# pearl-robot-lab/2HandedAfforder

Hardware: AMD Instinct MI355X
Metric: affordance frames/sec/GPU @1024^2, 32-tok prompt; mask IoU vs ref (higher is better)
Workload: dtype bf16; 1 GPU; BASELINE.json configs[2]: 2HandedAfforder-7B, 64 x 1024x1024 uint8 NHWC frames/step/GPU, 32-token prompt (T=291), 8 forced answer tokens with [SEG], KV-cached greedy decode, random-init weights; CLIP + SAM preprocessing of the uint8 frames on the device inside the step; parallelism=frame-sharded replicas x1 (no collective), hip_streams=2, fp32_decoder_tail=True, fp32_residual_stream=off, neck_f32=False, sam_chunk=16, sam_waits_for_prefill=False, decode_chain=False

## Files before the change

### 2handedafforder_amd/csrc/attention.hip

```cpp
#include "haff_common.h"

#include <type_traits>

namespace {

struct AttnArgs {
  const bf16_t *q = nullptr, *k = nullptr, *v = nullptr;
  bf16_t* o = nullptr;
  long q_sb = 0, q_sh = 0, q_st = 0;
  long k_sb = 0, k_sh = 0, k_st = 0;
  long v_sb = 0, v_sh = 0, v_st = 0;
  long o_sb = 0, o_sh = 0, o_st = 0;
  int B = 0, H = 0, Nq = 0, Nk = 0, d = 0;
  float scale = 0.f;
  int q_pos0 = 0;
  const float *relh = nullptr, *relw = nullptr;
  int S = 0;
  const int* nk_rows = nullptr;
  const bf16_t *knew = nullptr, *vnew = nullptr;
  const float* cos_sin = nullptr;
  const bf16_t *tab_h = nullptr, *tab_w = nullptr;
  float* lse = nullptr;
};
static_assert(std::is_trivially_copyable<AttnArgs>::value && sizeof(AttnArgs) == 240, "AttnArgs is passed to the kernels by value");

constexpr int QB = 128;
constexpr int KT = 64;
constexpr float LOG2E = 1.4426950408889634f;

typedef __attribute__((address_space(3))) bf16x4* lds_v4_ptr;


template <int DP, int BIAS, bool CAUSAL, int NDT = DP / 16, bool LSUM = false, bool FULL = false, bool F16 = false>
__global__ __launch_bounds__(256, 2) void attn_fwd_kernel(AttnArgs p) {
  using E = h16<F16>;
  static_assert(!FULL || (!CAUSAL && BIAS != 3), "FULL tiles only");
  constexpr int KSTRIDE = (DP * 2) % 64 == 32 ? DP * 2 : DP * 2 + 32;
  constexpr int VSTRIDE = DP * 2 + 32;
  constexpr int NCH = DP / 32;
  constexpr int CPR = DP / 8;
  constexpr int ND = NDT;
  constexpr int NKD = DP / 32;
  constexpr int SMAX = 32;
  constexpr int RSTRIDE = 2 * SMAX + 1;

  extern __shared__ __attribute__((aligned(16))) unsigned char smem_raw[];
  constexpr int STAGE_BYTES = KT * KSTRIDE + KT * VSTRIDE;
  unsigned char* sKV = smem_raw;
  float* sRel = reinterpret_cast<float*>(smem_raw + 2 * STAGE_BYTES);

  const int tid = threadIdx.x;
  const int lane = tid & 63;
  const int wave = tid >> 6;
  const int fr = lane & 15, fh = lane >> 4;
  const int nqb = (p.Nq + QB - 1) / QB;
  const int nbh = p.B * p.H;
  int bh_id, qblk;
  {
    const int id = blockIdx.x;
    if ((nbh & 7) == 0) {
      bh_id = (id & 7) + 8 * (id / (8 * nqb));
      qblk = (id >> 3) % nqb;
    } else {
      bh_id = id / nqb;
      qblk = id - bh_id * nqb;
    }
  }
  const int b = bh_id / p.H, h = bh_id - b * p.H;
  const int q0 = qblk * QB;
  const int Nk = p.nk_rows ? min(p.nk_rows[b], p.Nk) : p.Nk;

  const bf16_t* qb = p.q + (long)b * p.q_sb + (long)h * p.q_sh;
  const bf16_t* kb = p.k + (long)b * p.k_sb + (long)h * p.k_sh;
  const bf16_t* vb = p.v + (long)b * p.v_sb + (long)h * p.v_sh;

  const float sl2 = p.scale * LOG2E;
  bf16x8 qf[2][NKD];
  int qrow[2];
#pragma unroll
  for (int qt = 0; qt < 2; ++qt) {
    const int qi = q0 + wave * 32 + qt * 16 + fr;
    qrow[qt] = qi;
    const int qc = min(qi, p.Nq - 1);
#pragma unroll
    for (int kd = 0; kd < NKD; ++kd) {
      const int col = kd * 32 + fh * 8;
      uint4 r = make_uint4(0, 0, 0, 0);
      if (col < p.d) {
        float qv[8];
        load8h<F16>(qb + (long)qc * p.q_st + col, qv);
#pragma unroll
        for (int j = 0; j < 8; ++j) qv[j] *= sl2;
        r.x = E::pack2(qv[0], qv[1]); r.y = E::pack2(qv[2], qv[3]);
        r.z = E::pack2(qv[4], qv[5]); r.w = E::pack2(qv[6], qv[7]);
      }
      qf[qt][kd] = __builtin_bit_cast(bf16x8, r);
    }
  }

  const float inv_S = p.S > 0 ? 1.0f / (float)p.S : 0.f;
  float relw_r[2][4][4];
  const float* relh_row[2];
  if (BIAS == 2) {
    const long bh = (long)b * p.H + h;
#pragma unroll
    for (int qt = 0; qt < 2; ++qt) {
      const int qc = min(qrow[qt], p.Nq - 1);
      const float* rw = p.relw + (bh * p.Nq + qc) * p.S;
      relh_row[qt] = p.relh + (bh * p.Nq + qc) * p.S;
#pragma unroll
      for (int t = 0; t < 4; ++t) {
        float4 f = *reinterpret_cast<const float4*>(rw + 16 * t + 4 * fh);
        relw_r[qt][t][0] = f.x * LOG2E; relw_r[qt][t][1] = f.y * LOG2E;
        relw_r[qt][t][2] = f.z * LOG2E; relw_r[qt][t][3] = f.w * LOG2E;
      }
    }
  }
  float relh3[2][16], relw3[2][4];
  bool kw_ok[4];
  if (BIAS == 3) {
    const long bh = (long)b * p.H + h;
#pragma unroll
    for (int r = 0; r < 4; ++r) kw_ok[r] = (4 * fh + r) < p.S;
#pragma unroll
    for (int qt = 0; qt < 2; ++qt) {
      const int qc = min(qrow[qt], p.Nq - 1);
      const float* rh = p.relh + (bh * p.Nq + qc) * p.S;
      const float* rw = p.relw + (bh * p.Nq + qc) * p.S;
#pragma unroll
      for (int j = 0; j < 16; ++j) relh3[qt][j] = rh[min(j, p.S - 1)] * LOG2E;
#pragma unroll
      for (int r = 0; r < 4; ++r) relw3[qt][r] = rw[min(4 * fh + r, p.S - 1)] * LOG2E;
    }
  }
  if (BIAS == 1) {
    const long bh = (long)b * p.H + h;
    for (int i = tid; i < QB * 2 * p.S; i += 256) {
      const int ql = i / (2 * p.S);
      const int j = i - ql * 2 * p.S;
      const int qc = min(q0 + ql, p.Nq - 1);
      const float val = (j < p.S) ? p.relh[(bh * p.Nq + qc) * p.S + j] : p.relw[(bh * p.Nq + qc) * p.S + (j - p.S)];
      sRel[ql * RSTRIDE + j] = val * LOG2E;
    }
  }

  float relh_next[2] = {0.f, 0.f};
  if (BIAS == 2) {
    relh_next[0] = relh_row[0][0];
    relh_next[1] = relh_row[1][0];
  }

  int st_row[NCH], st_c[NCH];
#pragma unroll
  for (int i = 0; i < NCH; ++i) {
    const int id = tid + i * 256;
    st_row[i] = id / CPR;
    st_c[i] = id - st_row[i] * CPR;
  }
  uint4 kreg[NCH], vreg[NCH];
#pragma unroll
  for (int i = 0; i < NCH; ++i) kreg[i] = vreg[i] = make_uint4(0, 0, 0, 0);
  const bf16_t* kptr[NCH];
  const bf16_t* vptr[NCH];
  bool col_ok[NCH];
#pragma unroll
  for (int i = 0; i < NCH; ++i) {
    col_ok[i] = st_c[i] * 8 < p.d;
    kptr[i] = kb + (long)st_row[i] * p.k_st + st_c[i] * 8;
    vptr[i] = vb + (long)st_row[i] * p.v_st + st_c[i] * 8;
  }
  const long k_step = (long)KT * p.k_st, v_step = (long)KT * p.v_st;
  auto load_tile = [&](int kt) {
    const bool plain = FULL || ((BIAS != 3) && (kt * KT + KT <= Nk));
#pragma unroll
    for (int i = 0; i < NCH; ++i) {
      if (col_ok[i]) {
        if (plain) {
          kreg[i] = *reinterpret_cast<const uint4*>(kptr[i] + kt * k_step);
          vreg[i] = *reinterpret_cast<const uint4*>(vptr[i] + kt * v_step);
        } else {
          int key = kt * KT + st_row[i];
          if (BIAS == 3) key = min(key >> 4, p.S - 1) * p.S + min(key & 15, p.S - 1);
          key = min(key, Nk - 1);
          kreg[i] = *reinterpret_cast<const uint4*>(kb + (long)key * p.k_st + st_c[i] * 8);
          vreg[i] = *reinterpret_cast<const uint4*>(vb + (long)key * p.v_st + st_c[i] * 8);
        }
      }
    }
  };
  auto write_tile = [&](int buf) {
    unsigned char* wK = sKV + buf * STAGE_BYTES;
    unsigned char* wV = wK + KT * KSTRIDE;
#pragma unroll
    for (int i = 0; i < NCH; ++i) {
      if (col_ok[i]) {
        *reinterpret_cast<uint4*>(wK + st_row[i] * KSTRIDE + st_c[i] * 16) = kreg[i];
        *reinterpret_cast<uint4*>(wV + st_row[i] * VSTRIDE + st_c[i] * 16) = vreg[i];
      }
    }
  };
#pragma unroll
  for (int i = 0; i < NCH; ++i) {
    if (!col_ok[i]) {
      uint4 vpad = make_uint4(0, 0, 0, 0);
      if (LSUM && st_c[i] * 8 == p.d) vpad.x = F16 ? 0x3c00u : 0x3f80u;
#pragma unroll
      for (int b2 = 0; b2 < 2; ++b2) {
        unsigned char* wK = sKV + b2 * STAGE_BYTES;
        unsigned char* wV = wK + KT * KSTRIDE;
        *reinterpret_cast<uint4*>(wK + st_row[i] * KSTRIDE + st_c[i] * 16) = make_uint4(0, 0, 0, 0);
        *reinterpret_cast<uint4*>(wV + st_row[i] * VSTRIDE + st_c[i] * 16) = vpad;
      }
    }
  }

  f32x4 oacc[ND][2];
#pragma unroll
  for (int dt = 0; dt < ND; ++dt) {
    oacc[dt][0] = f32x4{0.f, 0.f, 0.f, 0.f};
    oacc[dt][1] = f32x4{0.f, 0.f, 0.f, 0.f};
  }
  float m_run[2] = {0.f, 0.f};
  float l_run[2] = {0.f, 0.f};

  int nkt = (Nk + KT - 1) / KT;
  if (BIAS == 3) nkt = (16 * p.S + KT - 1) / KT;
  if (CAUSAL) {
    const int last_q = min(q0 + QB - 1, p.Nq - 1);
    const int last_key = min(last_q + p.q_pos0, Nk - 1);
    nkt = min(nkt, last_key / KT + 1);
  }

  load_tile(0);
  write_tile(0);
  __syncthreads();
  for (int kt = 0; kt < nkt; ++kt) {
    const unsigned char* sK = sKV + (kt & 1) * STAGE_BYTES;
    const unsigned char* sV = sK + KT * KSTRIDE;
    float rh_cur[2] = {relh_next[0], relh_next[1]};
    if (BIAS == 2) asm volatile("" : "+v"(rh_cur[0]), "+v"(rh_cur[1]));
    if (kt + 1 < nkt) load_tile(kt + 1);

    f32x4 sacc[4][2];
#pragma unroll
    for (int qt = 0; qt < 2; ++qt) {
      float rh3[4] = {0.f, 0.f, 0.f, 0.f};
      if (BIAS == 3) {
#pragma unroll
        for (int j = 0; j < 4; ++j)
          rh3[j] = kt == 0 ? relh3[qt][j] : (kt == 1 ? relh3[qt][4 + j] : (kt == 2 ? relh3[qt][8 + j] : relh3[qt][12 + j]));
      }
      const float msub = m_run[qt];
      const float rhv = rh_cur[qt] * LOG2E - msub;
#pragma unroll
      for (int t = 0; t < 4; ++t) {
        if (BIAS == 2) sacc[t][qt] = f32x4{relw_r[qt][t][0] + rhv, relw_r[qt][t][1] + rhv, relw_r[qt][t][2] + rhv, relw_r[qt][t][3] + rhv};
        else if (BIAS == 3) {
          const float rb = rh3[t] - msub;
          sacc[t][qt] = f32x4{relw3[qt][0] + rb, relw3[qt][1] + rb, relw3[qt][2] + rb, relw3[qt][3] + rb};
        }
        else sacc[t][qt] = f32x4{-msub, -msub, -msub, -msub};
      }
      if (BIAS == 2 && kt + 1 < nkt) relh_next[qt] = relh_row[qt][kt + 1];
    }
#pragma unroll
    for (int kd = 0; kd < NKD; ++kd) {
#pragma unroll
      for (int t = 0; t < 4; ++t) {
        const bf16x8 kf = *reinterpret_cast<const bf16x8*>(sK + (16 * t + fr) * KSTRIDE + (kd * 4 + fh) * 16);
        sacc[t][0] = E::mfma16(kf, qf[0][kd], sacc[t][0]);
        sacc[t][1] = E::mfma16(kf, qf[1][kd], sacc[t][1]);
      }
    }

    bool need_mask = !FULL && (kt * KT + KT > Nk);
    if (CAUSAL) need_mask = need_mask || (kt * KT + KT - 1 > q0 + wave * 32 + p.q_pos0);
    int off_h[4][4], off_w[4][4];
    if (BIAS == 1) {
#pragma unroll
      for (int t = 0; t < 4; ++t)
#pragma unroll
        for (int r = 0; r < 4; ++r) {
          const int kc = min(kt * KT + 16 * t + 4 * fh + r, Nk - 1);
          const int kh = (int)(((float)kc + 0.5f) * inv_S);
          off_h[t][r] = kh;
          off_w[t][r] = p.S + kc - kh * p.S;
        }
    }
    bf16x8 pf[2][2];
#pragma unroll
    for (int qt = 0; qt < 2; ++qt) {
      const float* rel_q = sRel + (wave * 32 + qt * 16 + fr) * RSTRIDE;
      float mx = -1e30f;
#pragma unroll
      for (int t = 0; t < 4; ++t) {
#pragma unroll
        for (int r = 0; r < 4; ++r) {
          if (BIAS == 1) sacc[t][qt][r] += rel_q[off_h[t][r]] + rel_q[off_w[t][r]];
        }
      }
      if (BIAS == 3) {
#pragma unroll
        for (int t = 0; t < 4; ++t) {
          const bool row_ok = (4 * kt + t) < p.S;
#pragma unroll
          for (int r = 0; r < 4; ++r) sacc[t][qt][r] = (row_ok && kw_ok[r]) ? sacc[t][qt][r] : -INFINITY;
        }
      } else if (need_mask) {
#pragma unroll
        for (int t = 0; t < 4; ++t)
#pragma unroll
          for (int r = 0; r < 4; ++r) {
            const int key = kt * KT + 16 * t + 4 * fh + r;
            bool ok = key < Nk;
            if (CAUSAL) ok = ok && (key <= qrow[qt] + p.q_pos0);
            sacc[t][qt][r] = ok ? sacc[t][qt][r] : -INFINITY;
          }
      }
#pragma unroll
      for (int t = 0; t < 4; ++t) {
        mx = fmaxf(fmaxf(mx, sacc[t][qt][0]), sacc[t][qt][1]);
        mx = fmaxf(fmaxf(mx, sacc[t][qt][2]), sacc[t][qt][3]);
      }
      mx = fmaxf(mx, __shfl_xor(mx, 16, 64));
      mx = fmaxf(mx, __shfl_xor(mx, 32, 64));
      if (kt == 0 || __any(mx > 0.f)) {
        const float delta = kt == 0 ? fmaxf(mx, -1e30f) : fmaxf(mx, 0.f);
        const float alpha = kt == 0 ? 1.f : __builtin_amdgcn_exp2f(-delta);
        m_run[qt] += delta;
        const float shift = delta;
        l_run[qt] *= alpha;
#pragma unroll
        for (int dt = 0; dt < ND; ++dt) {
          oacc[dt][qt][0] *= alpha; oacc[dt][qt][1] *= alpha;
          oacc[dt][qt][2] *= alpha; oacc[dt][qt][3] *= alpha;
        }
#pragma unroll
        for (int t = 0; t < 4; ++t)
#pragma unroll
          for (int r = 0; r < 4; ++r) sacc[t][qt][r] -= shift;
      }
      float psum = 0.f;
#pragma unroll
      for (int t = 0; t < 4; ++t)
#pragma unroll
        for (int r = 0; r < 4; ++r) {
          const float e = __builtin_amdgcn_exp2f(sacc[t][qt][r]);
          sacc[t][qt][r] = e;
          if (!LSUM) psum += e;
        }
      if (!LSUM) l_run[qt] += psum;
#pragma unroll
      for (int ks = 0; ks < 2; ++ks) {
        uint4 u;
        u.x = E::pack2(sacc[2 * ks][qt][0], sacc[2 * ks][qt][1]);
        u.y = E::pack2(sacc[2 * ks][qt][2], sacc[2 * ks][qt][3]);
        u.z = E::pack2(sacc[2 * ks + 1][qt][0], sacc[2 * ks + 1][qt][1]);
        u.w = E::pack2(sacc[2 * ks + 1][qt][2], sacc[2 * ks + 1][qt][3]);
        pf[qt][ks] = __builtin_bit_cast(bf16x8, u);
      }
    }

    const int tr_q = fr >> 2, tr_p = fr & 3;
#pragma unroll
    for (int ks = 0; ks < 2; ++ks) {
#pragma unroll
      for (int dt = 0; dt < ND; ++dt) {
        const unsigned char* a0 = sV + (16 * (2 * ks) + 4 * fh + tr_q) * VSTRIDE + (16 * dt + 4 * tr_p) * 2;
        const unsigned char* a1 = a0 + 16 * VSTRIDE;
        const bf16x4 lo = __builtin_amdgcn_ds_read_tr16_b64_v4i16((lds_v4_ptr)(a0));
        const bf16x4 hi = __builtin_amdgcn_ds_read_tr16_b64_v4i16((lds_v4_ptr)(a1));
        const bf16x8 vf = __builtin_shufflevector(lo, hi, 0, 1, 2, 3, 4, 5, 6, 7);
        oacc[dt][0] = E::mfma16(vf, pf[0][ks], oacc[dt][0]);
        oacc[dt][1] = E::mfma16(vf, pf[1][ks], oacc[dt][1]);
      }
    }
    if (kt + 1 < nkt) write_tile((kt + 1) & 1);
    __syncthreads();
  }

  bf16_t* ob = p.o + (long)b * p.o_sb + (long)h * p.o_sh;
#pragma unroll
  for (int qt = 0; qt < 2; ++qt) {
    float l;
    if (LSUM) {
      l = __shfl(oacc[ND - 1][qt][0], fr, 64);
    } else {
      l = l_run[qt];
      l += __shfl_xor(l, 16, 64);
      l += __shfl_xor(l, 32, 64);
    }
    const float inv = 1.0f / l;
    if (p.lse && fh == 0 && qrow[qt] < p.Nq) p.lse[((long)b * p.H + h) * p.Nq + qrow[qt]] = m_run[qt] + __builtin_amdgcn_logf(l);
    if (qrow[qt] < p.Nq) {
#pragma unroll
      for (int dt = 0; dt < ND; ++dt) {
        const int col = 16 * dt + 4 * fh;
        if (col < p.d) {
          float v[4] = {oacc[dt][qt][0] * inv, oacc[dt][qt][1] * inv, oacc[dt][qt][2] * inv, oacc[dt][qt][3] * inv};
          store4h<F16>(ob + (long)qrow[qt] * p.o_st + col, v);
        }
      }
    }
  }
}

template <int DP, int BIAS, bool CAUSAL, int NDT = DP / 16, bool LSUM = false, bool FULL = false, bool F16 = false>
int launch_attn(const AttnArgs& p, hipStream_t s) {
  constexpr int KSTRIDE = (DP * 2) % 64 == 32 ? DP * 2 : DP * 2 + 32, VSTRIDE = DP * 2 + 32;
  size_t lds = 2 * ((size_t)KT * KSTRIDE + (size_t)KT * VSTRIDE);
  if (BIAS == 1) lds += (size_t)QB * (2 * 32 + 1) * sizeof(float);
  dim3 grid(((p.Nq + QB - 1) / QB) * p.H * p.B), block(256);
  hipLaunchKernelGGL((attn_fwd_kernel<DP, BIAS, CAUSAL, NDT, LSUM, FULL, F16>), grid, block, lds, s, p);
  return haff_check_launch();
}

constexpr int PPQ = 256;
constexpr int PP_D = 80, PP_CPR = PP_D / 8;
constexpr int PP_KSTR = PP_CPR * 16, PP_VSTR = PP_CPR * 16;
static_assert(PP_KSTR % 64 == 32, "K fragment reads are conflict-free for row strides of 32 mod 64 bytes");
constexpr int PP_KBYTES = KT * PP_KSTR, PP_VBYTES = KT * PP_VSTR;
constexpr int PP_KINS = PP_KBYTES / 1024, PP_VINS = PP_VBYTES / 1024;
constexpr int PP_NST = 4;
constexpr int PP_RSTR = KT + 1;
constexpr int PP_LDS = PP_NST * (PP_KBYTES + PP_VBYTES) + PPQ * PP_RSTR * 4;
constexpr float PP_LAZY = 40.f;
constexpr float PP_LAZY_F16 = 15.f;
static_assert(PP_KBYTES % 1024 == 0 && PP_VBYTES % 1024 == 0, "whole DMA instructions per tile");
static_assert(PP_LDS <= 160 * 1024, "LDS");

template <bool FUSED_REL, bool F16 = false>
__global__ __launch_bounds__(512, 1) void attn_global_pp_kernel(AttnArgs p) {
  using E = h16<F16>;
  constexpr int NKD = 3, ND = 5;
  extern __shared__ __attribute__((aligned(16))) unsigned char smem_raw[];
  typedef __attribute__((address_space(3))) unsigned char* lds_ptr;
  float* sRh = reinterpret_cast<float*>(smem_raw + PP_NST * (PP_KBYTES + PP_VBYTES));

  const int tid = threadIdx.x;
  const int lane = tid & 63;
  const int wave = __builtin_amdgcn_readfirstlane(tid >> 6);
  const int grp = wave >> 2;
  const int fr = lane & 15, fh = lane >> 4;
  const int nqb = p.Nq / PPQ;
  const int nbh = p.B * p.H;
  int bh_id, qblk;
  {
    const int id = blockIdx.x;
    if ((nbh & 15) == 0 && (p.H & 1) == 0) {
      const int x = id & 7, seq = id / (8 * nqb);
      bh_id = 16 * (seq >> 1) + 2 * x + (seq & 1);
      qblk = (id >> 3) % nqb;
    } else if ((nbh & 7) == 0) {
      bh_id = (id & 7) + 8 * (id / (8 * nqb));
      qblk = (id >> 3) % nqb;
    } else {
      bh_id = id / nqb;
      qblk = id - bh_id * nqb;
    }
  }
  const int b = bh_id / p.H, h = bh_id - b * p.H;
  const int q0 = qblk * PPQ;
  const bf16_t* qb = p.q + (long)b * p.q_sb + (long)h * p.q_sh;
  const bf16_t* kb = p.k + (long)b * p.k_sb + (long)h * p.k_sh;
  const long bh = (long)b * p.H + h;
  const int nkt = p.Nk / KT;

  auto fence_barrier_early = [&]() {
    __builtin_amdgcn_sched_barrier(0);
    __builtin_amdgcn_s_barrier();
    __builtin_amdgcn_sched_barrier(0);
  };
  constexpr int NINS = PP_KINS + PP_VINS;
  unsigned d_off[3];
  const unsigned v_minus_k = (unsigned)((p.v - p.k) * 2);
  int n_kins = 0, n_vins = 0;
#pragma unroll
  for (int i = 0; i < 3; ++i) {
    const int n = wave + 8 * i;
    unsigned off = 0;
    if (n < PP_KINS) {
      const int g = n * 64 + lane, row = g / PP_CPR, c = g - row * PP_CPR;
      off = (unsigned)(row * p.k_st * 2) + c * 16;
      ++n_kins;
    } else if (n < NINS) {
      const int g = (n - PP_KINS) * 64 + lane, row = g / PP_CPR, c = g - row * PP_CPR;
      off = v_minus_k + (unsigned)(row * p.v_st * 2) + c * 16;
      ++n_vins;
    }
    d_off[i] = off;
  }
  const unsigned k_step = (unsigned)(KT * p.k_st * 2), v_step = (unsigned)(KT * p.v_st * 2);
  const unsigned ldsK0 = (unsigned)(uintptr_t)(lds_ptr)smem_raw;
  const unsigned ldsV0 = ldsK0 + PP_NST * PP_KBYTES;
  auto issue = [&](int kt_k, int kt_v) -> int {
#pragma unroll
    for (int i = 0; i < 3; ++i) {
      const int n = wave + 8 * i;
      if (n < PP_KINS) {
        if (kt_k < nkt) {
          const unsigned m0v = ldsK0 + (kt_k % PP_NST) * PP_KBYTES + n * 1024;
          const unsigned off = d_off[i] + kt_k * k_step;
          asm volatile("s_mov_b32 m0, %2\n\ts_nop 0\n\tglobal_load_lds_dwordx4 %0, %1" ::"v"(off), "s"(kb), "s"(m0v) : "memory");
        }
      } else if (n < NINS) {
        if (kt_v < nkt) {
          const unsigned m0v = ldsV0 + (kt_v % PP_NST) * PP_VBYTES + (n - PP_KINS) * 1024;
          const unsigned off = d_off[i] + kt_v * v_step;
          asm volatile("s_mov_b32 m0, %2\n\ts_nop 0\n\tglobal_load_lds_dwordx4 %0, %1" ::"v"(off), "s"(kb), "s"(m0v) : "memory");
        }
      }
    }
    return (kt_k < nkt ? n_kins : 0) + (kt_v < nkt ? n_vins : 0);
  };
  const float sl2 = p.scale * LOG2E;
  bf16x8 qf[2][NKD];
  float relw_r[2][4][4];
  int qloc[2];
#pragma unroll
  for (int qt = 0; qt < 2; ++qt) {
    qloc[qt] = wave * 32 + qt * 16 + fr;
    const int qi = q0 + qloc[qt];
#pragma unroll
    for (int kd = 0; kd < NKD; ++kd) {
      const int col = kd * 32 + fh * 8;
      uint4 r = make_uint4(0, 0, 0, 0);
      if (col < PP_D) {
        float qv[8];
        load8h<F16>(qb + (long)qi * p.q_st + col, qv);
#pragma unroll
        for (int j = 0; j < 8; ++j) qv[j] *= sl2;
        r.x = E::pack2(qv[0], qv[1]); r.y = E::pack2(qv[2], qv[3]);
        r.z = E::pack2(qv[4], qv[5]); r.w = E::pack2(qv[6], qv[7]);
      }
      qf[qt][kd] = __builtin_bit_cast(bf16x8, r);
    }
  }
  if constexpr (FUSED_REL) {
    constexpr int SCR = KT + 4;
    static_assert(8 * 32 * SCR * 4 <= PP_NST * (PP_KBYTES + PP_VBYTES), "rel_w scratch fits the stage area");
    float* scr = reinterpret_cast<float*>(smem_raw) + wave * 32 * SCR;
    const int tok0 = q0 + wave * 32;
    const int qh = tok0 / KT, qwb = tok0 - qh * KT;
    const int nrow = 2 * KT - 2;
    bf16x8 qr[2][NKD];
#pragma unroll
    for (int qt = 0; qt < 2; ++qt)
#pragma unroll
      for (int kd = 0; kd < NKD; ++kd) {
        const int col = kd * 32 + fh * 8;
        uint4 r = make_uint4(0, 0, 0, 0);
        if (col < PP_D) r = *reinterpret_cast<const uint4*>(qb + (long)(q0 + qloc[qt]) * p.q_st + col);
        qr[qt][kd] = __builtin_bit_cast(bf16x8, r);
      }
    auto table_frag = [&](const bf16_t* tab, int row, int kd) {
      const int col = kd * 32 + fh * 8;
      uint4 r = make_uint4(0, 0, 0, 0);
      if (col < PP_D) r = *reinterpret_cast<const uint4*>(tab + (long)min(row, nrow) * PP_D + col);
      return __builtin_bit_cast(bf16x8, r);
    };
#pragma unroll
    for (int j = 0; j < 4; ++j) {
      f32x4 a0 = {0.f, 0.f, 0.f, 0.f}, a1 = {0.f, 0.f, 0.f, 0.f};
#pragma unroll
      for (int kd = 0; kd < NKD; ++kd) {
        const bf16x8 tf = table_frag(p.tab_h, qh + 16 * j + fr, kd);
// ... 387 lines not shown
        if (key == Nk - 1) { kr[u] = knew_bits; vr[u] = vnew_bits; }
      } else {
        kr[u] = *reinterpret_cast<const uint4*>(kb + (long)key * p.k_st);
        vr[u] = *reinterpret_cast<const uint4*>(vb + (long)key * p.v_st);
      }
    }
#pragma unroll
    for (int u = 0; u < DEC_UNROLL; ++u) {
      const int key = (it0 + u) * 4 + g;
      const unsigned kw[4] = {kr[u].x, kr[u].y, kr[u].z, kr[u].w};
      float s = 0.f;
#pragma unroll
      for (int j = 0; j < 4; ++j) {
        s = __builtin_fmaf(qv[2 * j], E::lo(kw[j]), s);
        s = __builtin_fmaf(qv[2 * j + 1], E::hi(kw[j]), s);
      }
      s = row16_sum(s);
      s = key < Nk ? s : -INFINITY;
      const float m_new = fmaxf(m_run, s);
      const float alpha = __builtin_amdgcn_exp2f(m_run - m_new);
      const float pr = __builtin_amdgcn_exp2f(s - m_new);
      m_run = m_new;
      l_run = l_run * alpha + pr;
      const unsigned vw[4] = {vr[u].x, vr[u].y, vr[u].z, vr[u].w};
#pragma unroll
      for (int j = 0; j < 4; ++j) {
        o[2 * j] = o[2 * j] * alpha + pr * E::lo(vw[j]);
        o[2 * j + 1] = o[2 * j + 1] * alpha + pr * E::hi(vw[j]);
      }
    }
  }
  float m_all = fmaxf(m_run, __shfl_xor(m_run, 16, 64));
  m_all = fmaxf(m_all, __shfl_xor(m_all, 32, 64));
  const float w = __builtin_amdgcn_exp2f(m_run - m_all);
  float l = l_run * w;
  l += __shfl_xor(l, 16, 64);
  l += __shfl_xor(l, 32, 64);
#pragma unroll
  for (int j = 0; j < 8; ++j) {
    float x = o[j] * w;
    x += __shfl_xor(x, 16, 64);
    x += __shfl_xor(x, 32, 64);
    o[j] = x;
  }
  if (!SPLIT) {
#pragma unroll
    for (int j = 0; j < 8; ++j) o[j] /= l;
    if (g == 0) store8h<F16>(p.o + (long)b * p.o_sb + (long)h * p.o_sh + c * 8, o);
    return;
  }
  if (g == 0) {
#pragma unroll
    for (int j = 0; j < 8; ++j) s_o[wave][c * 8 + j] = o[j];
    if (c == 0) { s_ml[wave][0] = m_all; s_ml[wave][1] = l; }
  }
  __syncthreads();
  if (wave == 0 && g == 0) {
    float M = s_ml[0][0];
#pragma unroll
    for (int w4 = 1; w4 < NW; ++w4) M = fmaxf(M, s_ml[w4][0]);
    float L = 0.f, acc[8] = {0.f, 0.f, 0.f, 0.f, 0.f, 0.f, 0.f, 0.f};
#pragma unroll
    for (int w4 = 0; w4 < NW; ++w4) {
      const float f = __builtin_amdgcn_exp2f(s_ml[w4][0] - M);
      L += s_ml[w4][1] * f;
#pragma unroll
      for (int j = 0; j < 8; ++j) acc[j] += s_o[w4][c * 8 + j] * f;
    }
#pragma unroll
    for (int j = 0; j < 8; ++j) acc[j] /= L;
    store8h<F16>(p.o + (long)b * p.o_sb + (long)h * p.o_sh + c * 8, acc);
  }
}

}

static AttnArgs attn_args(const void* q, long q_sb, long q_sh, long q_st,
                          const void* k, long k_sb, long k_sh, long k_st,
                          const void* v, long v_sb, long v_sh, long v_st,
                          void* o, long o_sb, long o_sh, long o_st,
                          int B, int H, int Nq, int Nk, int d, float scale) {
  AttnArgs p;
  p.q = reinterpret_cast<const bf16_t*>(q); p.q_sb = q_sb; p.q_sh = q_sh; p.q_st = q_st;
  p.k = reinterpret_cast<const bf16_t*>(k); p.k_sb = k_sb; p.k_sh = k_sh; p.k_st = k_st;
  p.v = reinterpret_cast<const bf16_t*>(v); p.v_sb = v_sb; p.v_sh = v_sh; p.v_st = v_st;
  p.o = reinterpret_cast<bf16_t*>(o); p.o_sb = o_sb; p.o_sh = o_sh; p.o_st = o_st;
  p.B = B; p.H = H; p.Nq = Nq; p.Nk = Nk; p.d = d; p.scale = scale;
  return p;
}

template <int BIAS, bool CAUSAL, bool F16>
static int launch_attn_dp(int dp, const AttnArgs& p, hipStream_t s) {
  switch (dp) {
    case 64: return launch_attn<64, BIAS, CAUSAL, 64 / 16, false, false, F16>(p, s);
    case 96: return launch_attn<96, BIAS, CAUSAL, 96 / 16, false, false, F16>(p, s);
    default:
      if constexpr (F16 && BIAS != 0) return HAFF_ERR_UNSUPPORTED;
      else return launch_attn<128, BIAS, CAUSAL, 128 / 16, false, false, F16>(p, s);
  }
}
template <int DP, bool F16>
static int launch_attn_rel(bool tile_is_row, const AttnArgs& p, hipStream_t s) {
  return tile_is_row ? launch_attn<DP, 2, false, DP / 16, false, false, F16>(p, s) : launch_attn<DP, 1, false, DP / 16, false, false, F16>(p, s);
}

template <bool ROPE, bool F16>
static int launch_attn_decode(const AttnArgs& p, hipStream_t s) {
  const int bh = p.B * p.H;
  if (bh <= 128) hipLaunchKernelGGL((attn_decode_kernel<true, ROPE, 16, F16>), dim3(bh), dim3(1024), 0, s, p);
  else if (bh <= 1024) hipLaunchKernelGGL((attn_decode_kernel<true, ROPE, 4, F16>), dim3(bh), dim3(256), 0, s, p);
  else hipLaunchKernelGGL((attn_decode_kernel<false, ROPE, 4, F16>), dim3((bh + 3) / 4), dim3(256), 0, s, p);
  return haff_check_launch();
}

template <bool F16 = false>
static int attention_bf16_impl(const void* q, long q_sb, long q_sh, long q_st,
                               const void* k, long k_sb, long k_sh, long k_st,
                               const void* v, long v_sb, long v_sh, long v_st,
                               void* o, long o_sb, long o_sh, long o_st,
                               int B, int H, int Nq, int Nk, int d, float scale,
                               int causal, int q_pos0,
                               const float* relh, const float* relw, int S, const int* nk_rows, void* stream,
                               float* lse = nullptr) {
  if (B <= 0 || H <= 0 || Nq <= 0 || Nk <= 0 || d <= 0 || d > 128 || (d & 7)) return HAFF_ERR_BAD_ARG;
  if (!haff_strides_ok(q_sb, q_sh, q_st, k_sb, k_sh, k_st, v_sb, v_sh, v_st, o_sb, o_sh, o_st, 7, 3)) return HAFF_ERR_BAD_ARG;
  const bool rel = relh != nullptr && relw != nullptr;
  if (rel && (causal || S <= 0 || (Nk % S) != 0)) return HAFF_ERR_BAD_ARG;
  if (F16 && rel && d > 96) return HAFF_ERR_UNSUPPORTED;
  AttnArgs p = attn_args(q, q_sb, q_sh, q_st, k, k_sb, k_sh, k_st, v, v_sb, v_sh, v_st, o, o_sb, o_sh, o_st, B, H, Nq, Nk, d, scale);
  p.q_pos0 = q_pos0;
  p.relh = relh;
  p.relw = relw;
  p.S = S;
  p.nk_rows = nk_rows;
  p.lse = lse;
  hipStream_t s = reinterpret_cast<hipStream_t>(stream);
  if (!lse && !rel && Nq == 1 && d == DEC_D && (!causal || q_pos0 >= Nk - 1) && (o_sh & 7) == 0 && (o_sb & 7) == 0 && haff_aligned(o))
    return launch_attn_decode<false, F16>(p, s);
  const int dp = d <= 64 ? 64 : (d <= 96 ? 96 : 128);
  if (rel) {
    const int mode = (S == 64) ? 2 : (S <= 16 && Nk == S * S ? 3 : 1);
    if (mode == 1 && S > 32) return HAFF_ERR_UNSUPPORTED;
    if (mode == 3) return launch_attn_dp<3, false, F16>(dp, p, s);
    if (dp == 64) return launch_attn_rel<64, F16>(mode == 2, p, s);
    if (mode == 2 && d == 80) {
      if (attn_global_pp_ok(p, false)) return launch_attn_global_pp<false, F16>(p, s);
      if ((Nq % 128) == 0 && (Nk % KT) == 0 && !nk_rows) return launch_attn<96, 2, false, 6, true, true, F16>(p, s);
      return launch_attn<96, 2, false, 6, true, false, F16>(p, s);
    }
    if (dp == 96) return launch_attn_rel<96, F16>(mode == 2, p, s);
    if constexpr (!F16) return launch_attn_rel<128, F16>(mode == 2, p, s);
    return HAFF_ERR_UNSUPPORTED;
  }
  return causal ? launch_attn_dp<0, true, F16>(dp, p, s) : launch_attn_dp<0, false, F16>(dp, p, s);
}

extern "C" int haff_attention_bf16(const void* q, long q_sb, long q_sh, long q_st,
                                   const void* k, long k_sb, long k_sh, long k_st,
                                   const void* v, long v_sb, long v_sh, long v_st,
                                   void* o, long o_sb, long o_sh, long o_st,
                                   int B, int H, int Nq, int Nk, int d, float scale,
                                   int causal, int q_pos0,
                                   const float* relh, const float* relw, int S, void* stream) {
  return attention_bf16_impl(q, q_sb, q_sh, q_st, k, k_sb, k_sh, k_st, v, v_sb, v_sh, v_st, o, o_sb, o_sh, o_st, B, H, Nq, Nk, d,
                             scale, causal, q_pos0, relh, relw, S, nullptr, stream);
}

extern "C" int haff_attention_f16(const void* q, long q_sb, long q_sh, long q_st,
                                  const void* k, long k_sb, long k_sh, long k_st,
                                  const void* v, long v_sb, long v_sh, long v_st,
                                  void* o, long o_sb, long o_sh, long o_st,
                                  int B, int H, int Nq, int Nk, int d, float scale,
                                  int causal, int q_pos0,
                                  const float* relh, const float* relw, int S, void* stream) {
  return attention_bf16_impl<true>(q, q_sb, q_sh, q_st, k, k_sb, k_sh, k_st, v, v_sb, v_sh, v_st, o, o_sb, o_sh, o_st, B, H, Nq,
                                   Nk, d, scale, causal, q_pos0, relh, relw, S, nullptr, stream);
}

static bool lse_args_ok(const void* q, const void* k, const void* v, const void* o, const float* lse, int causal, int q_pos0) {
  if (!q || !k || !v || !o || !lse) return false;
  if (!haff_aligned(q) || !haff_aligned(k) || !haff_aligned(v) || !haff_aligned(o, 8) || !haff_aligned(lse, 4)) return false;
  return !(causal && q_pos0 < 0);
}

extern "C" int haff_attention_lse_bf16(const void* q, long q_sb, long q_sh, long q_st,
                                       const void* k, long k_sb, long k_sh, long k_st,
                                       const void* v, long v_sb, long v_sh, long v_st,
                                       void* o, long o_sb, long o_sh, long o_st,
                                       int B, int H, int Nq, int Nk, int d, float scale, int causal, int q_pos0,
                                       float* lse, void* stream) {
  if (!lse_args_ok(q, k, v, o, lse, causal, q_pos0)) return HAFF_ERR_BAD_ARG;
  return attention_bf16_impl(q, q_sb, q_sh, q_st, k, k_sb, k_sh, k_st, v, v_sb, v_sh, v_st, o, o_sb, o_sh, o_st, B, H, Nq, Nk, d,
                             scale, causal, q_pos0, nullptr, nullptr, 0, nullptr, stream, lse);
}
extern "C" int haff_attention_lse_f16(const void* q, long q_sb, long q_sh, long q_st,
                                      const void* k, long k_sb, long k_sh, long k_st,
                                      const void* v, long v_sb, long v_sh, long v_st,
                                      void* o, long o_sb, long o_sh, long o_st,
                                      int B, int H, int Nq, int Nk, int d, float scale, int causal, int q_pos0,
                                      float* lse, void* stream) {
  if (!lse_args_ok(q, k, v, o, lse, causal, q_pos0)) return HAFF_ERR_BAD_ARG;
  return attention_bf16_impl<true>(q, q_sb, q_sh, q_st, k, k_sb, k_sh, k_st, v, v_sb, v_sh, v_st, o, o_sb, o_sh, o_st, B, H, Nq,
                                   Nk, d, scale, causal, q_pos0, nullptr, nullptr, 0, nullptr, stream, lse);
}

template <bool F16 = false>
static int global_attention_impl(const void* q, long q_sb, long q_sh, long q_st,
                                 const void* k, long k_sb, long k_sh, long k_st,
                                 const void* v, long v_sb, long v_sh, long v_st,
                                 void* o, long o_sb, long o_sh, long o_st,
                                 int B, int H, int S, int d, float scale,
                                 const void* tab_h, const void* tab_w, void* stream) {
  if (B <= 0 || H <= 0 || S <= 0 || d <= 0 || !tab_h || !tab_w) return HAFF_ERR_BAD_ARG;
  if (!haff_strides_ok(q_sb, q_sh, q_st, k_sb, k_sh, k_st, v_sb, v_sh, v_st, o_sb, o_sh, o_st, 7, 3)) return HAFF_ERR_BAD_ARG;
  AttnArgs p = attn_args(q, q_sb, q_sh, q_st, k, k_sb, k_sh, k_st, v, v_sb, v_sh, v_st, o, o_sb, o_sh, o_st, B, H, S * S, S * S, d, scale);
  p.S = S;
  p.tab_h = reinterpret_cast<const bf16_t*>(tab_h);
  p.tab_w = reinterpret_cast<const bf16_t*>(tab_w);
  if (!attn_global_pp_ok(p, true)) return HAFF_ERR_UNSUPPORTED;
  return launch_attn_global_pp<true, F16>(p, reinterpret_cast<hipStream_t>(stream));
}
extern "C" int haff_global_attention_bf16(const void* q, long q_sb, long q_sh, long q_st,
                                          const void* k, long k_sb, long k_sh, long k_st,
                                          const void* v, long v_sb, long v_sh, long v_st,
                                          void* o, long o_sb, long o_sh, long o_st,
                                          int B, int H, int S, int d, float scale,
                                          const void* tab_h, const void* tab_w, void* stream) {
  return global_attention_impl(q, q_sb, q_sh, q_st, k, k_sb, k_sh, k_st, v, v_sb, v_sh, v_st, o, o_sb, o_sh, o_st, B, H, S, d, scale,
                               tab_h, tab_w, stream);
}
extern "C" int haff_global_attention_f16(const void* q, long q_sb, long q_sh, long q_st,
                                         const void* k, long k_sb, long k_sh, long k_st,
                                         const void* v, long v_sb, long v_sh, long v_st,
                                         void* o, long o_sb, long o_sh, long o_st,
                                         int B, int H, int S, int d, float scale,
                                         const void* tab_h, const void* tab_w, void* stream) {
  return global_attention_impl<true>(q, q_sb, q_sh, q_st, k, k_sb, k_sh, k_st, v, v_sb, v_sh, v_st, o, o_sb, o_sh, o_st, B, H, S, d,
                                     scale, tab_h, tab_w, stream);
}

extern "C" int haff_attention_decode_rows_bf16(const void* q, long q_sb, long q_sh,
                                               const void* k, long k_sb, long k_sh, long k_st,
                                               const void* v, long v_sb, long v_sh, long v_st,
                                               void* o, long o_sb, long o_sh,
                                               int B, int H, int Nk, int d, float scale, const int* nk_rows, void* stream) {
  if (!nk_rows) return HAFF_ERR_BAD_ARG;
  return attention_bf16_impl(q, q_sb, q_sh, (long)H * d, k, k_sb, k_sh, k_st, v, v_sb, v_sh, v_st, o, o_sb, o_sh, (long)H * d, B, H, 1,
                             Nk, d, scale, 0, 0, nullptr, nullptr, 0, nk_rows, stream);
}

extern "C" int haff_attention_decode_rows_f16(const void* q, long q_sb, long q_sh,
                                              const void* k, long k_sb, long k_sh, long k_st,
                                              const void* v, long v_sb, long v_sh, long v_st,
                                              void* o, long o_sb, long o_sh,
                                              int B, int H, int Nk, int d, float scale, const int* nk_rows, void* stream) {
  if (!nk_rows) return HAFF_ERR_BAD_ARG;
  return attention_bf16_impl<true>(q, q_sb, q_sh, (long)H * d, k, k_sb, k_sh, k_st, v, v_sb, v_sh, v_st, o, o_sb, o_sh, (long)H * d,
                                   B, H, 1, Nk, d, scale, 0, 0, nullptr, nullptr, 0, nk_rows, stream);
}

template <bool F16 = false>
static int decode_attention_rope_rows_impl(const void* qkv, long ld, void* kcache, void* vcache, const float* cos_sin,
                                           void* out, int B, int H, int d, int Tmax, float scale, const int* nk_rows,
                                           void* stream) {
  if (B <= 0 || H <= 0 || d != DEC_D || Tmax <= 0 || !nk_rows || !cos_sin || (ld & 7)) return HAFF_ERR_BAD_ARG;
  if (!haff_aligned(qkv) || !haff_aligned(kcache) || !haff_aligned(vcache) || !haff_aligned(out)) return HAFF_ERR_BAD_ARG;
  const long hd = (long)H * d, cache = (long)Tmax * hd;
  AttnArgs p = attn_args(qkv,  ld,  d,  hd,
                         kcache,  cache,  d,  hd,
                         vcache,  cache,  d,  hd,
                         out,  hd,  d,  hd, B, H, 1, Tmax, d, scale);
  p.nk_rows = nk_rows;
  p.knew = p.q + hd;
  p.vnew = p.q + 2 * hd;
  p.cos_sin = cos_sin;
  return launch_attn_decode<true, F16>(p, reinterpret_cast<hipStream_t>(stream));
}
extern "C" int haff_decode_attention_rope_rows_bf16(const void* qkv, long ld, void* kcache, void* vcache, const float* cos_sin,
                                                    void* out, int B, int H, int d, int Tmax, float scale, const int* nk_rows,
                                                    void* stream) {
  return decode_attention_rope_rows_impl(qkv, ld, kcache, vcache, cos_sin, out, B, H, d, Tmax, scale, nk_rows, stream);
}
extern "C" int haff_decode_attention_rope_rows_f16(const void* qkv, long ld, void* kcache, void* vcache, const float* cos_sin,
                                                   void* out, int B, int H, int d, int Tmax, float scale, const int* nk_rows,
                                                   void* stream) {
  return decode_attention_rope_rows_impl<true>(qkv, ld, kcache, vcache, cos_sin, out, B, H, d, Tmax, scale, nk_rows, stream);
}

namespace {
template <typename T>
__global__ __launch_bounds__(256) void relpos_tables_kernel(const T* q, long q_sb, long q_sh, long q_st,
                                                          const float* tab_h, const float* tab_w,
                                                          float* relh, float* relw, int H, int S, int d) {
  extern __shared__ __attribute__((aligned(16))) unsigned char smem_raw[];
  float* sq = reinterpret_cast<float*>(smem_raw);
  const int N = S * S;
  const int QPB = 32;
  const int b = blockIdx.z, h = blockIdx.y, q0 = blockIdx.x * QPB;
  const T* qb = q + (long)b * q_sb + (long)h * q_sh;
  for (int i = threadIdx.x; i < QPB * d; i += 256) {
    const int ql = i / d, c = i - ql * d;
    const int qi = min(q0 + ql, N - 1);
    sq[ql * (d + 1) + c] = elem<T>::ld(qb + (long)qi * q_st + c);
  }
  __syncthreads();
  const long bh = (long)b * H + h;
// ... 164 lines not shown
```

Measured before the change: 113.3 frames/s.

## Add short-sequence attention variant with interleaved wave rows and per-tile skipping

Adds a SHORT specialization of the flash-attention kernel for Nq <= 512, used for causal d=128 (LLM prefill, T=291) and non-causal d=64. The first query block absorbs the remainder, and waves take interleaved 16-row slices, so a partial block does not leave whole waves idle. Per key tile, each wave skips MFMA work for row groups that are out of range or fully masked under causality. The intent is to cut wasted compute on padded and causally empty tiles, at the cost of branch divergence and extra template variants.

```diff
diff --git a/2handedafforder_amd/csrc/attention.hip b/2handedafforder_amd/csrc/attention.hip
--- a/2handedafforder_amd/csrc/attention.hip
+++ b/2handedafforder_amd/csrc/attention.hip
@@ -26,15 +26,17 @@
 
 constexpr int QB = 128;
 constexpr int KT = 64;
+constexpr int ATTN_SHORT_NQ = 512;
 constexpr float LOG2E = 1.4426950408889634f;
 
 typedef __attribute__((address_space(3))) bf16x4* lds_v4_ptr;
 
 
-template <int DP, int BIAS, bool CAUSAL, int NDT = DP / 16, bool LSUM = false, bool FULL = false, bool F16 = false>
+template <int DP, int BIAS, bool CAUSAL, int NDT = DP / 16, bool LSUM = false, bool FULL = false, bool F16 = false, bool SHORT = false>
 __global__ __launch_bounds__(256, 2) void attn_fwd_kernel(AttnArgs p) {
   using E = h16<F16>;
   static_assert(!FULL || (!CAUSAL && BIAS != 3), "FULL tiles only");
+  static_assert(!SHORT || (BIAS == 0 && !LSUM && !FULL), "SHORT: plain or causal scores only");
   constexpr int KSTRIDE = (DP * 2) % 64 == 32 ? DP * 2 : DP * 2 + 32;
   constexpr int VSTRIDE = DP * 2 + 32;
   constexpr int NCH = DP / 32;
@@ -67,7 +69,10 @@
     }
   }
   const int b = bh_id / p.H, h = bh_id - b * p.H;
-  const int q0 = qblk * QB;
+  const int q_first = p.Nq - (nqb - 1) * QB;
+  const int q0 = SHORT ? (qblk == 0 ? 0 : q_first + (qblk - 1) * QB) : qblk * QB;
+  const int qend = SHORT ? q_first + qblk * QB : p.Nq;
+  const int wave_u = SHORT ? __builtin_amdgcn_readfirstlane(wave) : wave;
   const int Nk = p.nk_rows ? min(p.nk_rows[b], p.Nk) : p.Nk;
 
   const bf16_t* qb = p.q + (long)b * p.q_sb + (long)h * p.q_sh;
@@ -79,7 +84,7 @@
   int qrow[2];
 #pragma unroll
   for (int qt = 0; qt < 2; ++qt) {
-    const int qi = q0 + wave * 32 + qt * 16 + fr;
+    const int qi = SHORT ? q0 + qt * 64 + wave * 16 + fr : q0 + wave * 32 + qt * 16 + fr;
     qrow[qt] = qi;
     const int qc = min(qi, p.Nq - 1);
 #pragma unroll
@@ -226,7 +231,7 @@
   int nkt = (Nk + KT - 1) / KT;
   if (BIAS == 3) nkt = (16 * p.S + KT - 1) / KT;
   if (CAUSAL) {
-    const int last_q = min(q0 + QB - 1, p.Nq - 1);
+    const int last_q = SHORT ? qend - 1 : min(q0 + QB - 1, p.Nq - 1);
     const int last_key = min(last_q + p.q_pos0, Nk - 1);
     nkt = min(nkt, last_key / KT + 1);
   }
@@ -241,6 +246,7 @@
     if (BIAS == 2) asm volatile("" : "+v"(rh_cur[0]), "+v"(rh_cur[1]));
     if (kt + 1 < nkt) load_tile(kt + 1);
 
+    if constexpr (!SHORT) {
     f32x4 sacc[4][2];
 #pragma unroll
     for (int qt = 0; qt < 2; ++qt) {
@@ -375,6 +381,111 @@
         oacc[dt][1] = E::mfma16(vf, pf[1][ks], oacc[dt][1]);
       }
     }
+    } else {
+    auto tile_math = [&](auto on0, auto on1) __attribute__((always_inline)) {
+      constexpr bool on[2] = {decltype(on0)::value, decltype(on1)::value};
+      f32x4 sacc[4][2];
+#pragma unroll
+      for (int qt = 0; qt < 2; ++qt) {
+        if (!on[qt]) continue;
+        const float msub = m_run[qt];
+#pragma unroll
+        for (int t = 0; t < 4; ++t) sacc[t][qt] = f32x4{-msub, -msub, -msub, -msub};
+      }
+#pragma unroll
+      for (int kd = 0; kd < NKD; ++kd) {
+#pragma unroll
+        for (int t = 0; t < 4; ++t) {
+          const bf16x8 kf = *reinterpret_cast<const bf16x8*>(sK + (16 * t + fr) * KSTRIDE + (kd * 4 + fh) * 16);
+          if (on[0]) sacc[t][0] = E::mfma16(kf, qf[0][kd], sacc[t][0]);
+          if (on[1]) sacc[t][1] = E::mfma16(kf, qf[1][kd], sacc[t][1]);
+        }
+      }
+      bool need_mask = kt * KT + KT > Nk;
+      if (CAUSAL) need_mask = need_mask || (kt * KT + KT - 1 > q0 + wave_u * 16 + p.q_pos0);
+      bf16x8 pf[2][2];
+#pragma unroll
+      for (int qt = 0; qt < 2; ++qt) {
+        if (!on[qt]) continue;
+        float mx = -1e30f;
+        if (need_mask) {
+#pragma unroll
+          for (int t = 0; t < 4; ++t)
+#pragma unroll
+            for (int r = 0; r < 4; ++r) {
+              const int key = kt * KT + 16 * t + 4 * fh + r;
+              bool ok = key < Nk;
+              if (CAUSAL) ok = ok && (key <= qrow[qt] + p.q_pos0);
+              sacc[t][qt][r] = ok ? sacc[t][qt][r] : -INFINITY;
+            }
+        }
+#pragma unroll
+        for (int t = 0; t < 4; ++t) {
+          mx = fmaxf(fmaxf(mx, sacc[t][qt][0]), sacc[t][qt][1]);
+          mx = fmaxf(fmaxf(mx, sacc[t][qt][2]), sacc[t][qt][3]);
+        }
+        mx = fmaxf(mx, __shfl_xor(mx, 16, 64));
+        mx = fmaxf(mx, __shfl_xor(mx, 32, 64));
+        if (kt == 0 || __any(mx > 0.f)) {
+          const float delta = kt == 0 ? fmaxf(mx, -1e30f) : fmaxf(mx, 0.f);
+          const float alpha = kt == 0 ? 1.f : __builtin_amdgcn_exp2f(-delta);
+          m_run[qt] += delta;
+          l_run[qt] *= alpha;
+#pragma unroll
+          for (int dt = 0; dt < ND; ++dt) {
+            oacc[dt][qt][0] *= alpha; oacc[dt][qt][1] *= alpha;
+            oacc[dt][qt][2] *= alpha; oacc[dt][qt][3] *= alpha;
+          }
+#pragma unroll
+          for (int t = 0; t < 4; ++t)
+#pragma unroll
+            for (int r = 0; r < 4; ++r) sacc[t][qt][r] -= delta;
+        }
+        float psum = 0.f;
+#pragma unroll
+        for (int t = 0; t < 4; ++t)
+#pragma unroll
+          for (int r = 0; r < 4; ++r) {
+            const float e = __builtin_amdgcn_exp2f(sacc[t][qt][r]);
+            sacc[t][qt][r] = e;
+            psum += e;
+          }
+        l_run[qt] += psum;
+#pragma unroll
+        for (int ks = 0; ks < 2; ++ks) {
+          uint4 u;
+          u.x = E::pack2(sacc[2 * ks][qt][0], sacc[2 * ks][qt][1]);
+          u.y = E::pack2(sacc[2 * ks][qt][2], sacc[2 * ks][qt][3]);
+          u.z = E::pack2(sacc[2 * ks + 1][qt][0], sacc[2 * ks + 1][qt][1]);
+          u.w = E::pack2(sacc[2 * ks + 1][qt][2], sacc[2 * ks + 1][qt][3]);
+          pf[qt][ks] = __builtin_bit_cast(bf16x8, u);
+        }
+      }
+      const int tr_q = fr >> 2, tr_p = fr & 3;
+#pragma unroll
+      for (int ks = 0; ks < 2; ++ks) {
+#pragma unroll
+        for (int dt = 0; dt < ND; ++dt) {
+          const unsigned char* a0 = sV + (16 * (2 * ks) + 4 * fh + tr_q) * VSTRIDE + (16 * dt + 4 * tr_p) * 2;
+          const unsigned char* a1 = a0 + 16 * VSTRIDE;
+          const bf16x4 lo = __builtin_amdgcn_ds_read_tr16_b64_v4i16((lds_v4_ptr)(a0));
+          const bf16x4 hi = __builtin_amdgcn_ds_read_tr16_b64_v4i16((lds_v4_ptr)(a1));
+          const bf16x8 vf = __builtin_shufflevector(lo, hi, 0, 1, 2, 3, 4, 5, 6, 7);
+          if (on[0]) oacc[dt][0] = E::mfma16(vf, pf[0][ks], oacc[dt][0]);
+          if (on[1]) oacc[dt][1] = E::mfma16(vf, pf[1][ks], oacc[dt][1]);
+        }
+      }
+    };
+    bool act[2];
+#pragma unroll
+    for (int qt = 0; qt < 2; ++qt) {
+      const int r0 = q0 + qt * 64 + wave_u * 16;
+      act[qt] = r0 < qend && (!CAUSAL || kt == 0 || kt * KT <= min(r0 + 15, qend - 1) + p.q_pos0);
+    }
+    if (act[0] && act[1]) tile_math(std::true_type{}, std::true_type{});
+    else if (act[0]) tile_math(std::true_type{}, std::false_type{});
+    else if (act[1]) tile_math(std::false_type{}, std::true_type{});
+    }
     if (kt + 1 < nkt) write_tile((kt + 1) & 1);
     __syncthreads();
   }
@@ -391,8 +502,8 @@
       l += __shfl_xor(l, 32, 64);
     }
     const float inv = 1.0f / l;
-    if (p.lse && fh == 0 && qrow[qt] < p.Nq) p.lse[((long)b * p.H + h) * p.Nq + qrow[qt]] = m_run[qt] + __builtin_amdgcn_logf(l);
-    if (qrow[qt] < p.Nq) {
+    if (p.lse && fh == 0 && qrow[qt] < qend) p.lse[((long)b * p.H + h) * p.Nq + qrow[qt]] = m_run[qt] + __builtin_amdgcn_logf(l);
+    if (qrow[qt] < qend) {
 #pragma unroll
       for (int dt = 0; dt < ND; ++dt) {
         const int col = 16 * dt + 4 * fh;
@@ -405,13 +516,13 @@
   }
 }
 
-template <int DP, int BIAS, bool CAUSAL, int NDT = DP / 16, bool LSUM = false, bool FULL = false, bool F16 = false>
+template <int DP, int BIAS, bool CAUSAL, int NDT = DP / 16, bool LSUM = false, bool FULL = false, bool F16 = false, bool SHORT = false>
 int launch_attn(const AttnArgs& p, hipStream_t s) {
   constexpr int KSTRIDE = (DP * 2) % 64 == 32 ? DP * 2 : DP * 2 + 32, VSTRIDE = DP * 2 + 32;
   size_t lds = 2 * ((size_t)KT * KSTRIDE + (size_t)KT * VSTRIDE);
   if (BIAS == 1) lds += (size_t)QB * (2 * 32 + 1) * sizeof(float);
   dim3 grid(((p.Nq + QB - 1) / QB) * p.H * p.B), block(256);
-  hipLaunchKernelGGL((attn_fwd_kernel<DP, BIAS, CAUSAL, NDT, LSUM, FULL, F16>), grid, block, lds, s, p);
+  hipLaunchKernelGGL((attn_fwd_kernel<DP, BIAS, CAUSAL, NDT, LSUM, FULL, F16, SHORT>), grid, block, lds, s, p);
   return haff_check_launch();
 }
 
@@ -1105,6 +1216,10 @@
     if constexpr (!F16) return launch_attn_rel<128, F16>(mode == 2, p, s);
     return HAFF_ERR_UNSUPPORTED;
   }
+  if (!lse && Nq <= ATTN_SHORT_NQ) {
+    if (causal && dp == 128) return launch_attn<128, 0, true, 128 / 16, false, false, F16, true>(p, s);
+    if (!causal && dp == 64) return launch_attn<64, 0, false, 64 / 16, false, false, F16, true>(p, s);
+  }
   return causal ? launch_attn_dp<0, true, F16>(dp, p, s) : launch_attn_dp<0, false, F16>(dp, p, s);
 }
 
```

Measured after the change: 113.3 frames/s. Within noise of the previous version (-0.0%).
